# philbull/FastBox

Hardware: AMD Instinct MI355X
Metric: 512^3 box realisations/sec (gen + log-normal + P(k)) (higher is better)
Workload: dtype f32; 1 GPU; 512^3 Gaussian box (device Philox4x32-10 noise, stand-in EH P(k), L=1000 Mpc) + log-normal transform + binned P(k), nbins=20; nsamp=512, parallelism=replicas x1, streams_per_gpu=2, warmup_steps_run=5, spin_up_steps=160, full=False

## Files before the change

fastbox_amd/_lib.py:

```python
import ctypes
import os
import subprocess

_HERE = os.path.dirname(os.path.abspath(__file__))
LIB_PATH = os.environ.get("FASTBOX_HIP_LIB") or os.path.join(_HERE, "lib", "libfastbox_hip.so")
CSRC = os.path.join(_HERE, "csrc")

c_void_p, c_int, c_double, c_size_t = ctypes.c_void_p, ctypes.c_int, ctypes.c_double, ctypes.c_size_t
c_u64, c_i64 = ctypes.c_uint64, ctypes.c_int64
P_double = ctypes.POINTER(ctypes.c_double)
P_i32 = ctypes.POINTER(ctypes.c_int32)

SIGNATURES = {
    "fb_version": (c_int, []),
    "fb_last_error": (ctypes.c_char_p, []),
    "fb_plan_create": (c_int, [ctypes.POINTER(c_void_p), c_int, c_double, c_double, c_double, c_int, c_int,
                               P_double, P_double, P_double, P_double]),
    "fb_plan_destroy": (c_int, [c_void_p]),
    "fb_half_pitch": (c_int, [c_void_p]),
    "fb_half_rows": (c_int, [c_void_p]),
    "fb_real_bytes": (c_i64, [c_void_p]),
    "fb_half_bytes": (c_i64, [c_void_p]),
    "fb_full_bytes": (c_i64, [c_void_p]),
    "fb_fft_c2c": (c_int, [c_void_p, c_void_p, c_int, c_double, c_void_p]),
# ... 157 lines not shown
    "fb_slab_z_pass": (c_int, [c_void_p, c_void_p, c_void_p, c_int, c_int, c_int, c_void_p, c_void_p]),
    "fb_slab_x_bin_chunk": (c_int, [c_void_p, c_void_p, c_int, c_int, c_int, c_int, c_int, c_int, c_void_p, c_void_p]),
    "fb_set_plane_batching": (c_int, [c_void_p, c_int, c_int]),
    "fb_set_pass_schedule": (c_int, [c_void_p, c_int, c_int, c_int]),
    "fb_set_tile_rows": (c_int, [c_void_p, c_int]),
    "fb_comm_unique_id": (c_int, [c_void_p]),
    "fb_comm_create": (c_int, [c_void_p, c_int, c_int, c_void_p]),
    "fb_comm_destroy": (c_int, [c_void_p]),
    "fb_comm_info": (c_int, [c_void_p, P_i32, P_i32, P_i32]),
    "fb_slab_exchange_begin": (c_int, [c_void_p, c_void_p, c_void_p, c_i64, c_void_p, P_i32]),
    "fb_slab_exchange_wait": (c_int, [c_void_p, c_int, c_void_p]),
    "fb_slab_exchange": (c_int, [c_void_p, c_void_p, c_void_p, c_i64, c_void_p]),
    "fb_allreduce_f64": (c_int, [c_void_p, c_void_p, c_int, c_int, c_void_p]),
    "fb_set_exp_shift": (c_int, [c_void_p, ctypes.c_double]),
    "fb_debug_pair_flush": (c_int, [c_i64]),
    "fb_debug_strided_pass": (c_int, [c_void_p, c_void_p, c_int, c_int, c_void_p]),
    "fb_debug_read_stamps": (c_int, [c_void_p, ctypes.POINTER(ctypes.c_longlong), c_i64]),
    "fb_profile_select": (c_int, [c_void_p, ctypes.c_uint]),
    "fb_profile_sample": (c_int, [c_void_p, c_int, ctypes.POINTER(c_i64)]),
    "fb_profile_start": (c_int, [c_void_p]),
    "fb_profile_stop": (c_int, [c_void_p, c_void_p, P_double, ctypes.POINTER(c_i64), c_int]),
    "fb_malloc": (c_int, [ctypes.POINTER(c_void_p), c_size_t]),
    "fb_free": (c_int, [c_void_p]),
    "fb_memcpy_h2d": (c_int, [c_void_p, c_void_p, c_size_t, c_void_p]),
    "fb_memcpy_d2h": (c_int, [c_void_p, c_void_p, c_size_t, c_void_p]),
    "fb_memcpy_d2d": (c_int, [c_void_p, c_void_p, c_size_t, c_void_p]),
    "fb_stream_create": (c_int, [ctypes.POINTER(c_void_p)]),
    "fb_stream_create_priority": (c_int, [ctypes.POINTER(c_void_p), c_int]),
    "fb_stream_destroy": (c_int, [c_void_p]),
    "fb_stream_sync": (c_int, [c_void_p]),
# ... 83 lines not shown
```

fastbox_amd/csrc/fb_api.hip:

```cpp
#include "../../include/fastbox_hip.h"
#include "fb_plan.h"
#include "fb_api_util.h"
#include "fb_kshell.h"
#include <dlfcn.h>
#include <rccl/rccl.h>
#include <algorithm>
#include <cmath>
#include <cstdio>
#include <cstdlib>
#include <cstring>
#include <vector>

static thread_local std::string g_last_error;

void fb_set_error(const std::string& msg) { g_last_error = msg; }

int fb_hip_check(hipError_t e, const char* what) {
    if (e == hipSuccess) return FB_OK;
    g_last_error = std::string(what) + ": " + hipGetErrorString(e);
    (void)hipGetLastError();
    return e == hipErrorOutOfMemory ? FB_ERR_NOMEM : FB_ERR_HIP;
}

namespace {
template <typename B, typename T> int upload(B& dst, const T* src, size_t n) {
    FB_TRY(dst.ensure(n * sizeof(T)));
    FB_HIP(hipMemcpy(dst, src, n * sizeof(T), hipMemcpyHostToDevice));
    return FB_OK;
}
template <typename T> int make_twiddles(FbBuf<>& out, int N) {
    std::vector<T> h((size_t)2 * N);
    for (int j = 0; j < N; ++j) {
        const long double a = -2.0L * 3.14159265358979323846264338327950288L * (long double)j / (long double)N;
        h[2 * (size_t)j] = (T)cosl(a);
        h[2 * (size_t)j + 1] = (T)sinl(a);
    }
    return upload(out, h.data(), h.size());
}
}

extern "C" {

int fb_version(void) { return 102; }
const char* fb_last_error(void) { return g_last_error.c_str(); }

int fb_device_count(int* count) {
    FB_REQUIRE(count, "null pointer");
    FB_HIP(hipGetDeviceCount(count));
    return FB_OK;
}

int fb_device_get(int* device) {
    FB_REQUIRE(device, "null pointer");
// ... 110 lines not shown
    FB_QUIESCE();
    p->amp_dense = nullptr;
    return FB_DISPATCH(p, fbi_set_amp_shells_f32(p, amp, nshell), fbi_set_amp_shells_f64(p, amp, nshell));
}
int fb_set_amplitude_sym(fb_plan* p, const double* amp, int64_t n) {
    FB_REQUIRE(p && amp, "null pointer");
    FB_USE_DEVICE(p);
    FB_QUIESCE();
    return FB_DISPATCH(p, fbi_set_amp_sym_f32(p, amp, n), fbi_set_amp_sym_f64(p, amp, n));
}
int fb_set_amplitude_dense(fb_plan* p, const void* amp_dev) {
    FB_REQUIRE(p && amp_dev, "null pointer");
    FB_USE_DEVICE(p);
    FB_QUIESCE();
    p->amp_dense = amp_dev;
    return FB_OK;
}
int fb_colour_noise(fb_plan* p, const void* re, const void* im, void* out, void* stream) {
    FB_REQUIRE(p && re && im && out, "null pointer");
    FB_USE_DEVICE(p);
    hipStream_t s = (hipStream_t)stream;
    return FB_DISPATCH(p, fbi_colour_noise_f32(p, re, im, out, s), fbi_colour_noise_f64(p, re, im, out, s));
}
int fb_colour_device(fb_plan* p, uint64_t seed, uint64_t realisation, void* out, void* stream) {
    FB_REQUIRE(p && out, "null pointer");
    FB_USE_DEVICE(p);
    hipStream_t s = (hipStream_t)stream;
    return FB_DISPATCH(p, fbi_colour_device_f32(p, seed, realisation, out, s),
                       fbi_colour_device_f64(p, seed, realisation, out, s));
}
// ... 577 lines not shown

int64_t fb_slab_half_bytes(const fb_plan* p, int nparts) {
    return (p && nparts > 0) ? (int64_t)(p->N / nparts) * p->NR * p->NZP * 2 * p->prec : 0;
}
int64_t fb_slab_kspace_bytes(const fb_plan* p, int nparts) {
    return (p && nparts > 0) ? (int64_t)p->N * (p->N / nparts) * p->NZP * 2 * p->prec : 0;
}

int fb_debug_strided_pass(fb_plan* p, void* half, int axis, int mode, void* stream) {
    FB_REQUIRE(p && half, "null pointer");
    FB_USE_DEVICE(p);
    hipStream_t s = (hipStream_t)stream;
    return FB_DISPATCH(p, fbi_debug_pass_f32(p, half, axis, mode, s), fbi_debug_pass_f64(p, half, axis, mode, s));
}

int fb_set_pass_schedule(fb_plan* p, int plain, int generator, int binning) {
    FB_REQUIRE(p, "null pointer");
    FB_REQUIRE(plain >= -1 && plain <= 1 && generator >= -1 && generator <= 1 && binning >= -1 && binning <= 1,
               "schedule: 0 (one workgroup per tile), 1 (resident workgroups) or -1 (by grid size)");
    p->pass_schedule[0] = plain; p->pass_schedule[1] = generator; p->pass_schedule[2] = binning;
    return FB_OK;
}
int fb_set_tile_rows(fb_plan* p, int bytes) {
    FB_REQUIRE(p, "null pointer");
    FB_REQUIRE(bytes == 0 || bytes == 64 || bytes == 128, "row segment of the strided passes' tiles: 0 (default), 64 or 128 bytes");
    p->wide_rows = bytes == 0 ? -1 : (bytes == 64 ? 0 : 7);
    return FB_OK;
}
int fb_set_exp_shift(fb_plan* p, double shift) {
    FB_REQUIRE(p, "null pointer");
// ... 120 lines not shown
```

fastbox_amd/csrc/fb_fft_kernels.h:

```cpp
#pragma once
#include <type_traits>
#include "fb_fft.h"
#include "fb_field_kernels.h"

namespace fb {

#ifndef FB_E16_FROM
#define FB_E16_FROM 2048
#endif
constexpr int strided_elems(int n) { return n >= FB_E16_FROM ? 16 : fb_min(8, n); }

#ifndef FB_TILE_LINE
#define FB_TILE_LINE 128
#endif
template <typename T> constexpr int tile_cols(int n) {
    return fb_max(fb_max(2, fb_min(FB_TILE_LINE / (2 * (int)sizeof(T)),
                                   (n >= FB_E16_FROM ? (sizeof(T) == 8 ? 65536 : 131072) : 65536) / (n * 2 * (int)sizeof(T)))),
                  64 / (n / strided_elems(n)));
}

template <typename T> constexpr int strided_wg_per_cu(int n) {
    const int tile = n * tile_cols<T>(n) * 2 * (int)sizeof(T), nt = tile_cols<T>(n) * (n / strided_elems(n));
    return fb_max(1, fb_min(2048 / nt, tile > 81920 ? 1 : tile > 36864 ? 2 : 4));
}
// ... 57 lines not shown
    long long stride;
    long long outer_stride;
    int ncols;
    T scale;
    int ntx;
    int ntiles;
    int drop_io;
    int wide;
    int ntx_shift;
    long long out_outer_stride;
    long long blk_stride;
    int blk_in, blk_out, blk_shift;
    int packed;
    int tile0;
    long long out_stride;
};

template <typename T> struct StridedOp {
    KGeom g;
    AmpSrc<T> amp;
    RngKey key;
    const int* thr;
    const double* bins;
    double* partial;
    long long partial_stride;
    cx<T>* plane_out;
    int nbins, namb, store;
    int outer0;
    int vel_on, vel_comp;
    double vel_fac;
// ... 102 lines not shown
#pragma unroll
        for (int r = 0; r < 4; ++r)
            if (r * 64 < op.nbins) {
                int th;
                if constexpr (PERSIST) th = lthr[r * 64 + (tid & 63)];
                else th = thrv[r];
                b += __builtin_popcountll(__ballot(th <= n2));
            }
        return b;
    };
    [[maybe_unused]] const int rot_rows = (int)gridDim.x >= a.ntx ? (int)gridDim.x / a.ntx : 1;
    auto place = [&](int id, int& bx, int& by) {
        const bool p2 = a.ntx_shift >= 0;
        bx = p2 ? (id & (a.ntx - 1)) : id % a.ntx;
        by = p2 ? (id >> a.ntx_shift) : id / a.ntx;
#ifndef FB_NO_TILE_ROTATE
        int rot = bx + by;
        if constexpr (PERSIST) rot += by / rot_rows;
        bx = p2 ? (rot & (a.ntx - 1)) : rot % a.ntx;
#endif
#ifndef FB_NO_XCD_PAIR
        if constexpr (TZ * sizeof(cx<T>) < 128) {
            constexpr int LPT = 128 / (TZ * (int)sizeof(cx<T>)), G = 8 * LPT;
            const int lg = bx % G;
            if (bx - lg + G <= a.ntx) bx = (bx - lg) + LPT * (lg % 8) + lg / 8;
        }
#endif
        bx += a.tile0;
    };
    int tile_id = blockIdx.x;
#ifndef FB_GEN_PARK
#define FB_GEN_PARK 16
#endif
// ... 66 lines not shown
                if (has_plane) {
                    asm volatile("");
                    plane = (kz == 0) || (kz == H);
                    flip = plane && ky > H;
                    kyd = flip ? N - ky : ky;
                }
                cx<T> wl[ACC ? NJ : 1], wh[ACC ? NJ : 1];
                auto lo = [&](int j) -> cx<T>& { if constexpr (ACC) return wl[j - J0]; else return v[j]; };
                auto hi = [&](int j) -> cx<T>& { if constexpr (ACC) return wh[j - J0]; else return v[j + E2]; };
                T A0[NJ], A1[NJ];
                auto A0v = [&](int j) -> T { return A0[j - J0]; };
                auto A1v = [&](int j) -> T { return A1[j - J0]; };
                {
                    const T pf = (T)0.70710678118654752440;
                    if (op.amp.sym) {
                        const long long sym_step = (long long)TPL * (H + 1) * op.g.NZP;
                        const T* sym0 = op.amp.sym + ((long long)t * (H + 1) + amy) * op.g.NZP + kz;
                        const T* sym1 = op.amp.sym + ((long long)(H - t) * (H + 1) + amy) * op.g.NZP + kz;
#pragma unroll
                        for (int j = J0; j < J0 + NJ; ++j) {
#ifdef FB_EXPERIMENT_NOAMP
                            A0[j - J0] = pf; A1[j - J0] = pf;
#else
                            A0[j - J0] = sym0[j * sym_step] * pf;
                            A1[j - J0] = sym1[-j * sym_step] * pf;
#endif
                        }
                    } else if (op.amp.shell) {
                        const int c2 = my * my + kz * kz;
#pragma unroll
                        for (int j = J0; j < J0 + NJ; ++j) {
                            const int kx = t + j * TPL, mh = kx - H;
                            A0[j - J0] = op.amp.shell[kx * kx + c2] * pf;
// ... 780 lines not shown
```

fastbox_amd/csrc/fb_fft_launch.inc:

```
#include <cstdlib>
#include <cstring>
#include "fb_plan.h"
#include "fb_fft_kernels.h"
#include "fb_fft_generic.h"

namespace {

using namespace fb;
typedef FB_REAL real_t;
typedef cx<real_t> cplx_t;

template <typename K> int set_lds(K kernel, size_t bytes) {
    if (bytes > 65536)
        FB_HIP(hipFuncSetAttribute(reinterpret_cast<const void*>(kernel),
                                   hipFuncAttributeMaxDynamicSharedMemorySize, (int)bytes));
    return FB_OK;
}

KGeom fft_geom(const fb_plan* p) { return KGeom{p->axis2, p->ksc, p->kpar, p->N, p->NZV, p->NZP, p->NR}; }
int gen_amplitude(const fb_plan* p, StridedOp<real_t>& op) {
    op.amp.shell = (p->amp_dense || p->amp_sym_only) ? nullptr : p->amp_shell.as<const real_t>();
    op.amp.dense = p->amp_sym_only ? nullptr : reinterpret_cast<const real_t*>(p->amp_dense);
    op.amp.sym = (op.amp.shell || p->amp_sym_only) ? p->amp_sym.as<const real_t>() : nullptr;
    if (!op.amp.shell && !op.amp.dense && !op.amp.sym) { fb_set_error("amplitude table not set (fb_set_amplitude_*)"); return FB_ERR_STATE; }
    return FB_OK;
}

template <int N, int MODE, int PERSIST, bool BLK>
int launch_strided_npb(fb_plan* p, const StridedArgs<real_t>& a, int nouter, int sign, StridedOp<real_t>& op,
                       hipStream_t s) {
    constexpr bool SPLIT = strided_split<real_t>(N, MODE, BLK);
    constexpr int E = strided_elems_of<real_t>(N, MODE, BLK), TPL = N / E, TZ = tile_cols_of<real_t>(N, MODE, BLK);
    constexpr int NW = (TZ * TPL + 63) / 64;
    size_t lds = (size_t)N * TZ * (SPLIT ? sizeof(real_t) : sizeof(cplx_t)) + (size_t)N * sizeof(cplx_t);
    if (smode_bins(MODE)) lds += (size_t)NW * 2 * op.nbins * sizeof(double) + (size_t)((op.nbins + 63) & ~63) * sizeof(int);
    StridedArgs<real_t> b = a;
    b.ntx = a.ntx ? a.ntx : (a.ncols + TZ - 1) / TZ;
    b.ntiles = b.ntx * nouter;
    b.ntx_shift = -1;
    for (int q = 0; q < 30; ++q) if ((1 << q) == b.ntx) b.ntx_shift = q;
    b.wide = ((long long)(E - 1) * TPL * a.stride * (long long)sizeof(cplx_t) >= 0xE0000000LL) ? 1 : 0;
    b.drop_io = p->debug_no_mem;
    auto pick = [&]() {
#ifndef FB_CSIGN_FROM
#define FB_CSIGN_FROM (1 << 30)
#endif
        if constexpr (MODE == SMODE_PLAIN && (strided_row128<real_t>(N, MODE, BLK) || N >= (FB_CSIGN_FROM)))
            return sign < 0 ? k_fft_strided<real_t, N, MODE, PERSIST, BLK, -1> : k_fft_strided<real_t, N, MODE, PERSIST, BLK, +1>;
        else return k_fft_strided<real_t, N, MODE, PERSIST, BLK>;
    };
    auto kernel = pick();
    int r = set_lds(kernel, lds);
    if (r) return r;
    int nblk = b.ntiles;
    if (PERSIST) {
        static thread_local int per_cu = 0;
        static thread_local size_t per_cu_lds = 0;
// ... 630 lines not shown
}

int FB_CAT(fbi_debug_pass_, FB_SUFFIX)(fb_plan* p, void* half, int axis, int mode, hipStream_t s) {
    const int N = p->N;
    cplx_t* h = reinterpret_cast<cplx_t*>(half);
    const bool packed = use_packed(p) && mode % 10 != 2;
    StridedArgs<real_t> a = axis == 0 ? half_x(p, h, packed) : half_y(p, h, packed);
    StridedOp<real_t> op = {};
    op.g = fft_geom(p);
    p->debug_no_mem = (mode >= 10);
    mode %= 10;
    struct Reset { fb_plan* q; ~Reset() { q->debug_no_mem = 0; } } reset{p};
    if (mode == 1) {
        op.amp.shell = p->amp_shell.as<const real_t>();
        op.amp.dense = nullptr;
        op.amp.sym = p->amp_sym.as<const real_t>();
        if (!op.amp.shell) { fb_set_error("amplitude shells not set"); return FB_ERR_STATE; }
#ifdef FB_STAMPS
        {
            int r = p->bin_partials.ensure(((size_t)N * 64 * 32 + 4096) * sizeof(double));
            if (r) return r;
            op.bins = p->bin_partials;
        }
#endif
        return launch_strided<SMODE_GEN>(p, N, a, N, +1, op, s);
    }
    if (mode == 2) {
        if (!p->nbins || !p->use_thr) { fb_set_error("bins not set"); return FB_ERR_STATE; }
        op.thr = p->thr; op.bins = p->bins; op.nbins = p->nbins; op.namb = p->namb; op.store = 0;
        for (int q = 0; q < 8; ++q) op.amb[q] = p->amb[q];
        return launch_strided<SMODE_BIN>(p, N, a, N, -1, op, s);
// ... 121 lines not shown
    r = slab_blocking(ao, p, nxl, nparts, true);
    if (r) return r;
    return launch_plain(p, N, ao, nxl, -1, s);
}

int FB_CAT(fbi_slab_x_pass_, FB_SUFFIX)(fb_plan* p, void* kslab, int nyl, int sign, hipStream_t s) {
    return launch_plain(p, p->N, slab_x(p, reinterpret_cast<cplx_t*>(kslab), nyl), nyl, sign, s);
}

int FB_CAT(fbi_slab_x_generate_, FB_SUFFIX)(fb_plan* p, void* kslab, int nyl, int ky0, uint64_t seed, uint64_t real,
                                            hipStream_t s) {
    StridedOp<real_t> op = {};
    op.g = fft_geom(p);
    op.amp.shell = p->amp_shell.as<const real_t>();
    if (!op.amp.shell || p->amp_dense) { fb_set_error("slab generation needs shell amplitudes (cubic box)"); return FB_ERR_STATE; }
    op.amp.sym = p->amp_sym.as<const real_t>();
    op.key.k[0] = (uint32_t)seed; op.key.k[1] = (uint32_t)(seed >> 32);
    op.key.k[2] = (uint32_t)real; op.key.k[3] = (uint32_t)(real >> 32);
    op.outer0 = ky0;
    return launch_strided<SMODE_GEN>(p, p->N, slab_x(p, reinterpret_cast<cplx_t*>(kslab), nyl), nyl, +1, op, s);
}

int FB_CAT(fbi_slab_x_bin_, FB_SUFFIX)(fb_plan* p, void* kslab, int nyl, int ky0, double* results, hipStream_t s) {
    if (!p->nbins || !p->use_thr) { fb_set_error("fused P(k) needs shell thresholds (fb_set_bins with thr)"); return FB_ERR_STATE; }
    const int nb = p->nbins;
    StridedOp<real_t> op = {};
    op.g = fft_geom(p);
    op.thr = p->thr; op.bins = p->bins; op.nbins = nb; op.namb = p->namb; op.store = 0; op.outer0 = ky0;
    for (int q = 0; q < 8; ++q) op.amb[q] = p->amb[q];
    int r = launch_strided<SMODE_BIN>(p, p->N, slab_x(p, reinterpret_cast<cplx_t*>(kslab), nyl), nyl, -1, op, s);
    if (r) return r;
// ... 15 lines not shown
int slab_blocking_chunk(StridedArgs<real_t>& a, const fb_plan* p, int nxl, int nparts, long long W, bool out_side) {
    const int N = p->N, E = strided_elems(N);
    int m = E / nparts, shift = 0;
    if (nparts < 1 || m * nparts != E) { fb_set_error("fused slab exchange needs the rank count to divide the points per thread"); return FB_ERR_UNSUPPORTED; }
    while ((1 << shift) < m) ++shift;
    const long long nyl = N / nparts;
    a.blk_shift = shift;
    a.blk_stride = (long long)nxl * nyl * W;
    if (out_side) { a.blk_out = 1; a.out_stride = W; a.out_outer_stride = nyl * W; }
    else { a.blk_in = 1; a.out_stride = p->NZP; a.out_outer_stride = (long long)p->NR * p->NZP; a.stride = W; a.outer_stride = nyl * W; }
    return FB_OK;
}
}

int FB_CAT(fbi_slab_tile_cols_, FB_SUFFIX)(const fb_plan* p) { return slab_tz(p->N); }

int FB_CAT(fbi_slab_x_generate_chunk_, FB_SUFFIX)(fb_plan* p, void* kchunk, int nyl, int ky0, uint64_t seed, uint64_t real,
                                                  int tile0, int ntile, hipStream_t s) {
    const int TZ = slab_tz(p->N);
    const long long W = (long long)ntile * TZ;
    StridedOp<real_t> op = {};
    op.g = fft_geom(p);
    op.amp.shell = p->amp_shell.as<const real_t>();
    if (!op.amp.shell || p->amp_dense) { fb_set_error("slab generation needs shell amplitudes (cubic box)"); return FB_ERR_STATE; }
    op.amp.sym = p->amp_sym.as<const real_t>();
    op.key.k[0] = (uint32_t)seed; op.key.k[1] = (uint32_t)(seed >> 32);
    op.key.k[2] = (uint32_t)real; op.key.k[3] = (uint32_t)(real >> 32);
    op.outer0 = ky0;
    cplx_t* k = reinterpret_cast<cplx_t*>(kchunk) - (long long)tile0 * TZ;
    StridedArgs<real_t> a{k, k, p->tw.as<const cplx_t>(), (long long)nyl * W, W, p->NZV, (real_t)1};
    a.ntx = ntile; a.tile0 = tile0;
    return launch_strided<SMODE_GEN>(p, p->N, a, nyl, +1, op, s);
}

int FB_CAT(fbi_slab_y_inverse_chunk_, FB_SUFFIX)(fb_plan* p, const void* recv_chunk, void* half_local, int nxl, int nparts,
                                                 int tile0, int ntile, hipStream_t s) {
    const int TZ = slab_tz(p->N);
    const long long W = (long long)ntile * TZ;
    cplx_t* h = reinterpret_cast<cplx_t*>(half_local);
    StridedArgs<real_t> a = slab_y(p, h);
// ... 92 lines not shown
```

fastbox_amd/csrc/fb_field_kernels.h:

```cpp
#pragma once
#include "fb_dev.h"
#include "fb_fft.h"
#include "fb_kshell.h"
#include "fb_rng.h"

namespace fb {

__device__ __forceinline__ int mirror_of(int i, int N) { return i == 0 ? 0 : N - i; }

struct KGeom {
    const double* axis2;
    const double* ksc;
    const double* kpar;
    int N, NZV, NZP;
    int NR;
};

__device__ __forceinline__ void fb_sincospi(float x, float* s, float* c) { sincospif(x, s, c); }
__device__ __forceinline__ void fb_sincospi(double x, double* s, double* c) { sincospi(x, s, c); }
__device__ __forceinline__ void fb_sincos(float x, float* s, float* c) { sincosf(x, s, c); }
__device__ __forceinline__ void fb_sincos(double x, double* s, double* c) { sincos(x, s, c); }

__device__ __forceinline__ double kmag_exact(const KGeom& g, int i, int j, int l) {
#pragma clang fp contract(off)
// ... 11 lines not shown
}

template <typename T> __device__ __forceinline__ T nan_to_num(T v) {
    if (v != v) return (T)0;
    if (sizeof(T) == 4) { if (v > (T)3.4028234663852886e38) return (T)3.4028234663852886e38;
                          if (v < (T)-3.4028234663852886e38) return (T)-3.4028234663852886e38; }
    else { if (v > (T)1.7976931348623157e308) return (T)1.7976931348623157e308;
           if (v < (T)-1.7976931348623157e308) return (T)-1.7976931348623157e308; }
    return v;
}

template <typename T> struct AmpSrc {
    const T* shell;
    const T* dense;
    const T* sym;
};
template <typename T>
__global__ void k_build_amp_sym(const T* __restrict__ shell, T* __restrict__ sym, int N, int NZP) {
    const int M = (N >> 1) + 1;
    const int c = blockIdx.x * blockDim.x + threadIdx.x;
    const int b = blockIdx.y, a = blockIdx.z;
    if (c >= NZP) return;
    sym[((long long)a * M + b) * NZP + c] = c < M ? shell[a * a + b * b + c * c] : (T)0;
}
template <typename T>
__device__ __forceinline__ T amp_at(const AmpSrc<T>& a, const KGeom& g, int i, int j, int l) {
    if (a.shell) return a.shell[shell_of(i, j, l, g.N)];
    if (a.sym) {
        const int mi = mode_of(i, g.N), mj = mode_of(j, g.N), ml = mode_of(l, g.N);
        const int M = (g.N >> 1) + 1;
        return a.sym[((long long)(mi < 0 ? -mi : mi) * M + (mj < 0 ? -mj : mj)) * g.NZP + (ml < 0 ? -ml : ml)];
    }
    return a.dense[((long long)i * g.NR + j) * g.NZP + l];
}

template <typename T>
__global__ void k_colour_noise(const T* __restrict__ re, const T* __restrict__ im, cx<T>* __restrict__ out,
                               AmpSrc<T> amp, KGeom g) {
    const int N = g.N;
    const int l = blockIdx.x * blockDim.x + threadIdx.x;
    const int j = blockIdx.y, i = blockIdx.z;
    if (l >= g.NZV) return;
    const long long a = ((long long)i * N + j) * N + l;
    const long long b = ((long long)mirror_of(i, N) * N + mirror_of(j, N)) * N + mirror_of(l, N);
    const T A = (T)0.5 * amp_at(amp, g, i, j, l);
    out[((long long)i * g.NR + j) * g.NZP + l] = cx<T>{A * (re[a] + re[b]), A * (im[a] - im[b])};
// ... 1322 lines not shown
```

fastbox_amd/csrc/fb_field_launch.inc:

```
#include <algorithm>
#include <cmath>
#include <cstdlib>
#include "fb_plan.h"
#include "fb_api_util.h"
#include "fb_field_kernels.h"
#include <vector>

namespace {
using namespace fb;
typedef FB_REAL real_t;
typedef cx<real_t> cplx_t;

KGeom geom(const fb_plan* p) { return KGeom{p->axis2, p->ksc, p->kpar, p->N, p->NZV, p->NZP, p->NR}; }
BinGeom bin_geom(const fb_plan* p) {
    BinGeom b;
    b.bins = p->bins; b.thr = p->use_thr ? p->thr : nullptr; b.nbins = p->nbins; b.namb = p->namb;
    for (int q = 0; q < 8; ++q) b.amb[q] = p->amb[q];
    return b;
}
dim3 mode_grid(const fb_plan* p, int nz, int bs) { return dim3((nz + bs - 1) / bs, p->N, p->N); }
RngKey rng_key(uint64_t seed, uint64_t real) {
    RngKey k;
    k.k[0] = (uint32_t)seed; k.k[1] = (uint32_t)(seed >> 32); k.k[2] = (uint32_t)real; k.k[3] = (uint32_t)(real >> 32);
    return k;
}
dim3 row_grid(const fb_plan* p) {
    return dim3((unsigned)(((long long)p->N * p->N + FB_ROW_GROUPS - 1) / FB_ROW_GROUPS));
}
int mode_block(int nz) {
    int best = 64;
    for (int bs = 128; bs <= 256; bs <<= 1)
        if ((nz + bs - 1) / bs * bs <= (nz + best - 1) / best * best) best = bs;
    return best;
}

int amp_src(const fb_plan* p, AmpSrc<real_t>& a) {
    a.shell = p->amp_shell.as<const real_t>();
    a.dense = reinterpret_cast<const real_t*>(p->amp_dense);
    a.sym = p->amp_sym.as<const real_t>();
    if (a.dense) a.shell = nullptr;
    if (p->amp_sym_only) { a.shell = nullptr; a.dense = nullptr; }
    if (!a.shell && !a.dense && !a.sym) { fb_set_error("amplitude table not set (fb_set_amplitude_*)"); return FB_ERR_STATE; }
    return FB_OK;
}
}

#define FB_CAT2(a, b) a##b
#define FB_CAT(a, b) FB_CAT2(a, b)
#define FBI(name) FB_CAT(FB_CAT(fbi_, name), FB_CAT(_, FB_SUFFIX))

int FBI(set_amp_shells)(fb_plan* p, const double* amp, int64_t n) {
    std::vector<real_t> tmp((size_t)n);
    for (int64_t q = 0; q < n; ++q) tmp[(size_t)q] = (real_t)amp[q];
    FB_TRY(p->amp_shell.reset());
    FB_TRY(p->amp_shell.ensure((size_t)n * sizeof(real_t)));
    FB_HIP(hipMemcpy(p->amp_shell, tmp.data(), (size_t)n * sizeof(real_t), hipMemcpyHostToDevice));
    p->nshell = n;
    p->amp_sym_only = 0;
    const int N = p->N, M = N / 2 + 1;
    if (const char* e = getenv("FB_NO_AMP_SYM")) if (e[0] == '1') {
        return p->amp_sym.reset();
    }
    if (n < (int64_t)3 * (N / 2) * (N / 2) + 1) { fb_set_error("shell table shorter than 3 (N/2)^2 + 1"); return FB_ERR_INVALID; }
    FB_TRY(p->amp_sym.ensure((size_t)M * M * p->NZP * sizeof(real_t)));
    hipLaunchKernelGGL((k_build_amp_sym<real_t>), dim3((p->NZP + 63) / 64, M, M), dim3(64), 0, 0,
                       p->amp_shell.as<const real_t>(), p->amp_sym.as<real_t>(), N, p->NZP);
    FB_LAUNCH_CHECK("k_build_amp_sym");
    FB_HIP(hipDeviceSynchronize());
    return FB_OK;
}

int FBI(set_amp_sym)(fb_plan* p, const double* amp, int64_t n) {
    const int N = p->N, M = N / 2 + 1;
    if (n != (int64_t)M * M * M) { fb_set_error("expected (N/2+1)^3 amplitudes"); return FB_ERR_INVALID; }
    std::vector<real_t> tmp((size_t)M * M * p->NZP, (real_t)0);
    for (int a = 0; a < M; ++a)
        for (int b = 0; b < M; ++b)
            for (int c = 0; c < M; ++c)
                tmp[((size_t)a * M + b) * p->NZP + c] = (real_t)amp[((size_t)a * M + b) * M + c];
    FB_TRY(p->amp_sym.ensure(tmp.size() * sizeof(real_t)));
    FB_HIP(hipMemcpy(p->amp_sym, tmp.data(), tmp.size() * sizeof(real_t), hipMemcpyHostToDevice));
    p->amp_sym_only = 1;
    p->amp_dense = nullptr;
    return FB_OK;
}

int FBI(colour_noise)(fb_plan* p, const void* re, const void* im, void* out, hipStream_t s) {
    AmpSrc<real_t> a;
    int r = amp_src(p, a);
    if (r) return r;
    const int bs = mode_block(p->NZV);
    { FbProfScope _ps(p, FBK_COLOUR, s);
    hipLaunchKernelGGL((k_colour_noise<real_t>), mode_grid(p, p->NZV, bs), dim3(bs), 0, s,
                       (const real_t*)re, (const real_t*)im, (cplx_t*)out, a, geom(p)); }
    FB_LAUNCH_CHECK("k_colour_noise");
    return FB_OK;
// ... 434 lines not shown
```

fastbox_amd/csrc/fb_plan.h:

```cpp
#pragma once
#include <hip/hip_runtime.h>
#include <stdint.h>
#include "fb_keyed_cache.h"
#include <string>
#include <vector>

#define FB_OK 0
#define FB_ERR_INVALID -1
#define FB_ERR_HIP -2
#define FB_ERR_UNSUPPORTED -3
#define FB_ERR_NOMEM -4
#define FB_ERR_STATE -5
#define FB_ERR_RCCL -6

void fb_set_error(const std::string& msg);
int fb_hip_check(hipError_t e, const char* what);
#define FB_HIP(x) do { int _r = fb_hip_check((x), #x); if (_r) return _r; } while (0)
#define FB_TRY(x) do { const int _r = (x); if (_r) return _r; } while (0)
#define FB_LAUNCH_CHECK(name) do { int _r = fb_hip_check(hipGetLastError(), name); if (_r) return _r; } while (0)

template <typename T = void> struct FbBuf {
    T* ptr = nullptr;
    size_t cap = 0;
    FbBuf() = default;
// ... 6 lines not shown
    int ensure(size_t need) { return cap >= need ? FB_OK : grow(need); }
    int reset() {
        T* q = ptr;
        ptr = nullptr; cap = 0;
        if (q) FB_HIP(hipFree(q));
        return FB_OK;
    }
private:
    __attribute__((noinline)) int grow(size_t need) {
        FB_TRY(reset());
        FB_HIP(hipMalloc(reinterpret_cast<void**>(&ptr), need));
        cap = need;
        return FB_OK;
    }
};

struct fb_comm;

struct fb_cyl_rows {
    int nb = 0;
    FbBuf<int> rows_dev;
    std::vector<int> off;
    std::vector<double> sumk;
    bool has0 = false;
};

struct fb_plan {
    fb_comm* comm = nullptr;
    int N = 0;
    int generic = 0;
// ... 13 lines not shown
    int cubic = 0;

    FbBuf<> tw;
    FbBuf<double> axis2;
    FbBuf<double> kpar;
    FbBuf<double> ksc;
    FbBuf<double> zgrid;

    FbBuf<> amp_shell;
    int64_t nshell = 0;
    const void* amp_dense = nullptr;
    FbBuf<> work;
    FbBuf<double> eig_work;
    FbBuf<double> kperp_tab;
    int amp_sym_only = 0;
    FbBuf<> amp_sym;

    FbBuf<double> bins;
    int nbins = 0;
    FbBuf<int> thr;
    int use_thr = 0;
    int namb = 0;
    int amb[8] = {0, 0, 0, 0, 0, 0, 0, 0};
    FbBuf<unsigned long long> counts;
    double counts_host[256];
    FbBuf<double> partials;
    int prow = 0;
    FbBuf<double> scratch;
    FbBuf<double> bin_partials;
    long long bin_rows = 0;
    long long bin_rows_main = 0;
// ... 129 lines not shown
                                double scale, hipStream_t s); \
    int fbi_power_fused_##sfx(fb_plan* p, const void* real_in, void* work_half, int pre_exp, int store, \
                              double* results, hipStream_t s); \
    int fbi_debug_pass_##sfx(fb_plan* p, void* half, int axis, int mode, hipStream_t s); \
    int fbi_realise_begin_##sfx(fb_plan* p, uint64_t seed, uint64_t real, void* work_half, hipStream_t s); \
    int fbi_realise_finish_##sfx(fb_plan* p, void* work_half, void* real_out, double scale, hipStream_t s); \
    int fbi_power_from_pending_##sfx(fb_plan* p, void* work_half, void* real_out, double scale, int pre_exp, \
                                     double* results, hipStream_t s); \
    int fbi_slab_forward_local_##sfx(fb_plan* p, const void* real_local, void* half_local, int nxl, int pre_exp, \
                                     double* expsum, hipStream_t s); \
    int fbi_slab_inverse_local_##sfx(fb_plan* p, void* half_local, void* real_local, int nxl, double scale, hipStream_t s); \
    int fbi_slab_x_pass_##sfx(fb_plan* p, void* kslab, int nyl, int sign, hipStream_t s); \
    int fbi_slab_x_generate_##sfx(fb_plan* p, void* kslab, int nyl, int ky0, uint64_t seed, uint64_t real, hipStream_t s); \
    int fbi_slab_x_bin_##sfx(fb_plan* p, void* kslab, int nyl, int ky0, double* results, hipStream_t s); \
    int fbi_slab_tile_cols_##sfx(const fb_plan* p); \
    int fbi_slab_x_generate_chunk_##sfx(fb_plan* p, void* kchunk, int nyl, int ky0, uint64_t seed, uint64_t real, int tile0, \
                                        int ntile, hipStream_t s); \
    int fbi_slab_y_inverse_chunk_##sfx(fb_plan* p, const void* recv_chunk, void* half_local, int nxl, int nparts, int tile0, \
                                       int ntile, hipStream_t s); \
    int fbi_slab_y_forward_chunk_##sfx(fb_plan* p, const void* half_local, void* send_chunk, int nxl, int nparts, int tile0, \
                                       int ntile, hipStream_t s); \
    int fbi_slab_z_pass_##sfx(fb_plan* p, void* half_local, void* real_local, int nxl, int which, double scale, int pre_exp, \
                              double* expsum, hipStream_t s); \
    int fbi_slab_x_bin_chunk_##sfx(fb_plan* p, void* kchunk, int nyl, int ky0, int tile0, int ntile, int first, int last, \
                                   double* results, hipStream_t s);
FB_DECL(f32)
FB_DECL(f64)
int fbi_bin_count(fb_plan* p, hipStream_t s);
int fbi_slab_permute(fb_plan* p, const void* in, void* out, int nxl, int nparts, int pack, hipStream_t s);
```

include/fastbox_hip.h:

```cpp
#ifndef FASTBOX_HIP_H
#define FASTBOX_HIP_H

#include <stddef.h>
#include <stdint.h>

#ifdef __cplusplus
extern "C" {
#endif

#define FB_OK 0
#define FB_ERR_INVALID -1
#define FB_ERR_HIP -2
#define FB_ERR_UNSUPPORTED -3
#define FB_ERR_NOMEM -4
#define FB_ERR_STATE -5
#define FB_ERR_RCCL -6

typedef struct fb_plan fb_plan;

int fb_version(void);
const char* fb_last_error(void);

int fb_plan_create(fb_plan** plan, int N, double Lx, double Ly, double Lz, int precision, int device,
                   const double* axis2, const double* ksc, const double* kpar, const double* zgrid);
// ... 320 lines not shown
int fb_comm_unique_id(void* id128);
int fb_comm_create(fb_plan* plan, int world, int rank, const void* id128);
int fb_comm_destroy(fb_plan* plan);
int fb_comm_info(const fb_plan* plan, int* world, int* rank, int* rccl_version);
int fb_slab_exchange_begin(fb_plan* plan, const void* send, void* recv, int64_t bytes_per_peer, void* stream, int* ticket);
int fb_slab_exchange_wait(fb_plan* plan, int ticket, void* stream);
int fb_slab_exchange(fb_plan* plan, const void* send, void* recv, int64_t bytes_per_peer, void* stream);
int fb_allreduce_f64(fb_plan* plan, double* data_dev, int count, int op, void* stream);

int fb_set_plane_batching(fb_plan* plan, int planes, int streams);
int fb_set_pass_schedule(fb_plan* plan, int plain, int generator, int binning);
int fb_set_tile_rows(fb_plan* plan, int bytes);
int fb_set_exp_shift(fb_plan* plan, double shift);
int fb_debug_strided_pass(fb_plan* plan, void* half, int axis, int mode, void* stream);
int fb_debug_pair_flush(int64_t pairs);
int fb_debug_read_stamps(fb_plan* plan, long long* host, int64_t count);

int fb_malloc(void** dev_ptr, size_t bytes);
int fb_free(void* dev_ptr);
int fb_memcpy_h2d(void* dst_dev, const void* src_host, size_t bytes, void* stream);
int fb_memcpy_d2h(void* dst_host, const void* src_dev, size_t bytes, void* stream);
int fb_memcpy_d2d(void* dst_dev, const void* src_dev, size_t bytes, void* stream);
int fb_stream_create(void** stream);
int fb_stream_create_priority(void** stream, int priority);
int fb_stream_destroy(void* stream);
int fb_stream_sync(void* stream);
int fb_stream_wait_stream(void* waiter, void* signaller);
int fb_device_count(int* count);
int fb_device_get(int* device);
int fb_device_set(int device);
// ... 6 lines not shown
```

Before: 1051 boxes/s.

## Block amplitude symmetry table by tile columns, pair mirrored generator rows, share tables

Reorders the symmetric amplitude table into blocks of z-columns matched to the generator tile width, so that the mirrored t and H-t lookups hit contiguous short runs. The generator also schedules tile rows q and N-q in adjacent groups of eight tiles, so both mirror halves of a row reuse the same amplitude block in cache. A process-wide registry, keyed by hash, deduplicates identical amplitude tables across plans (for example across replicas), which saves device memory and L2 footprint. The cost is a more complex indexing scheme, a host-side hash of the shell table, and a new scheduling path that only runs when its divisibility conditions are met.

```diff
diff --git a/fastbox_amd/_lib.py b/fastbox_amd/_lib.py
--- a/fastbox_amd/_lib.py
+++ b/fastbox_amd/_lib.py
@@ -195,6 +195,7 @@
     "fb_allreduce_f64": (c_int, [c_void_p, c_void_p, c_int, c_int, c_void_p]),
     "fb_set_exp_shift": (c_int, [c_void_p, ctypes.c_double]),
     "fb_debug_pair_flush": (c_int, [c_i64]),
+    "fb_debug_amp_tables": (c_int, [ctypes.POINTER(c_i64)]),
     "fb_debug_strided_pass": (c_int, [c_void_p, c_void_p, c_int, c_int, c_void_p]),
     "fb_debug_read_stamps": (c_int, [c_void_p, ctypes.POINTER(ctypes.c_longlong), c_i64]),
     "fb_profile_select": (c_int, [c_void_p, ctypes.c_uint]),
diff --git a/fastbox_amd/csrc/fb_api.hip b/fastbox_amd/csrc/fb_api.hip
--- a/fastbox_amd/csrc/fb_api.hip
+++ b/fastbox_amd/csrc/fb_api.hip
@@ -37,6 +37,11 @@
     }
     return upload(out, h.data(), h.size());
 }
+}
+
+FbSharedRegistry<fb_amp_table>& fb_amp_registry() {
+    static FbSharedRegistry<fb_amp_table>* r = new FbSharedRegistry<fb_amp_table>();
+    return *r;
 }
 
 extern "C" {
@@ -177,6 +182,7 @@
     FB_USE_DEVICE(p);
     FB_QUIESCE();
     p->amp_dense = amp_dev;
+    if (!p->amp_sym_only) p->amp_sym.reset();
     return FB_OK;
 }
 int fb_colour_noise(fb_plan* p, const void* re, const void* im, void* out, void* stream) {
@@ -784,6 +790,12 @@
     return FB_DISPATCH(p, fbi_debug_pass_f32(p, half, axis, mode, s), fbi_debug_pass_f64(p, half, axis, mode, s));
 }
 
+int fb_debug_amp_tables(int64_t* tables) {
+    FB_REQUIRE(tables, "null pointer");
+    *tables = (int64_t)fb_amp_registry().live();
+    return FB_OK;
+}
+
 int fb_set_pass_schedule(fb_plan* p, int plain, int generator, int binning) {
     FB_REQUIRE(p, "null pointer");
     FB_REQUIRE(plain >= -1 && plain <= 1 && generator >= -1 && generator <= 1 && binning >= -1 && binning <= 1,
diff --git a/fastbox_amd/csrc/fb_fft_kernels.h b/fastbox_amd/csrc/fb_fft_kernels.h
--- a/fastbox_amd/csrc/fb_fft_kernels.h
+++ b/fastbox_amd/csrc/fb_fft_kernels.h
@@ -95,6 +95,7 @@
     int packed;
     int tile0;
     long long out_stride;
+    int pair_rows;
 };
 
 template <typename T> struct StridedOp {
@@ -227,9 +228,21 @@
         const bool p2 = a.ntx_shift >= 0;
         bx = p2 ? (id & (a.ntx - 1)) : id % a.ntx;
         by = p2 ? (id >> a.ntx_shift) : id / a.ntx;
+        [[maybe_unused]] int rk = by, rks = by;
+#ifndef FB_NO_GEN_MIRROR_PAIR
+        if constexpr (MODE == SMODE_GEN) {
+            if (a.pair_rows) {
+                const int u = ((id >> 4) << 3) | (id & 7), w = (id >> 3) & 1;
+                const int q = p2 ? (u >> a.ntx_shift) : u / a.ntx;
+                bx = p2 ? (u & (a.ntx - 1)) : u % a.ntx;
+                by = q ? (w ? N - q : q) : (w ? N / 2 : 0);
+                rk = q; rks = 2 * q;
+            }
+        }
+#endif
 #ifndef FB_NO_TILE_ROTATE
-        int rot = bx + by;
-        if constexpr (PERSIST) rot += by / rot_rows;
+        int rot = bx + rk;
+        if constexpr (PERSIST) rot += rks / rot_rows;
         bx = p2 ? (rot & (a.ntx - 1)) : rot % a.ntx;
 #endif
 #ifndef FB_NO_XCD_PAIR
@@ -326,9 +339,12 @@
                 {
                     const T pf = (T)0.70710678118654752440;
                     if (op.amp.sym) {
-                        const long long sym_step = (long long)TPL * (H + 1) * op.g.NZP;
-                        const T* sym0 = op.amp.sym + ((long long)t * (H + 1) + amy) * op.g.NZP + kz;
-                        const T* sym1 = op.amp.sym + ((long long)(H - t) * (H + 1) + amy) * op.g.NZP + kz;
+                        const int bs = op.amp.sym_bs;
+                        const long long sym_step = (long long)TPL << bs;
+                        const long long blk = ((long long)amy * (op.g.NZP >> bs) + (kz >> bs)) * (H + 1);
+                        const int kzl = kz & ((1 << bs) - 1);
+                        const T* sym0 = op.amp.sym + (((blk + t) << bs) + kzl);
+                        const T* sym1 = op.amp.sym + (((blk + (H - t)) << bs) + kzl);
 #pragma unroll
                         for (int j = J0; j < J0 + NJ; ++j) {
 #ifdef FB_EXPERIMENT_NOAMP
diff --git a/fastbox_amd/csrc/fb_fft_launch.inc b/fastbox_amd/csrc/fb_fft_launch.inc
--- a/fastbox_amd/csrc/fb_fft_launch.inc
+++ b/fastbox_amd/csrc/fb_fft_launch.inc
@@ -21,7 +21,8 @@
 int gen_amplitude(const fb_plan* p, StridedOp<real_t>& op) {
     op.amp.shell = (p->amp_dense || p->amp_sym_only) ? nullptr : p->amp_shell.as<const real_t>();
     op.amp.dense = p->amp_sym_only ? nullptr : reinterpret_cast<const real_t*>(p->amp_dense);
-    op.amp.sym = (op.amp.shell || p->amp_sym_only) ? p->amp_sym.as<const real_t>() : nullptr;
+    op.amp.sym = (op.amp.shell || p->amp_sym_only) ? p->sym<real_t>() : nullptr;
+    op.amp.sym_bs = p->sym_bs();
     if (!op.amp.shell && !op.amp.dense && !op.amp.sym) { fb_set_error("amplitude table not set (fb_set_amplitude_*)"); return FB_ERR_STATE; }
     return FB_OK;
 }
@@ -41,6 +42,7 @@
     for (int q = 0; q < 30; ++q) if ((1 << q) == b.ntx) b.ntx_shift = q;
     b.wide = ((long long)(E - 1) * TPL * a.stride * (long long)sizeof(cplx_t) >= 0xE0000000LL) ? 1 : 0;
     b.drop_io = p->debug_no_mem;
+    b.pair_rows = (MODE == SMODE_GEN && nouter == N && op.outer0 == 0 && b.ntiles % 16 == 0) ? 1 : 0;
     auto pick = [&]() {
 #ifndef FB_CSIGN_FROM
 #define FB_CSIGN_FROM (1 << 30)
@@ -701,7 +703,8 @@
     if (mode == 1) {
         op.amp.shell = p->amp_shell.as<const real_t>();
         op.amp.dense = nullptr;
-        op.amp.sym = p->amp_sym.as<const real_t>();
+        op.amp.sym = p->sym<real_t>();
+        op.amp.sym_bs = p->sym_bs();
         if (!op.amp.shell) { fb_set_error("amplitude shells not set"); return FB_ERR_STATE; }
 #ifdef FB_STAMPS
         {
@@ -853,7 +856,8 @@
     op.g = fft_geom(p);
     op.amp.shell = p->amp_shell.as<const real_t>();
     if (!op.amp.shell || p->amp_dense) { fb_set_error("slab generation needs shell amplitudes (cubic box)"); return FB_ERR_STATE; }
-    op.amp.sym = p->amp_sym.as<const real_t>();
+    op.amp.sym = p->sym<real_t>();
+    op.amp.sym_bs = p->sym_bs();
     op.key.k[0] = (uint32_t)seed; op.key.k[1] = (uint32_t)(seed >> 32);
     op.key.k[2] = (uint32_t)real; op.key.k[3] = (uint32_t)(real >> 32);
     op.outer0 = ky0;
@@ -899,6 +903,16 @@
 }
 
 int FB_CAT(fbi_slab_tile_cols_, FB_SUFFIX)(const fb_plan* p) { return slab_tz(p->N); }
+int FB_CAT(fbi_gen_tile_cols_, FB_SUFFIX)(const fb_plan* p) {
+    if (p->generic) return 0;
+    switch (p->N) {
+#define FB_GEN_TZ_CASE(N_) case N_: return tile_cols_of<real_t>(N_, SMODE_GEN, false);
+        FB_GEN_TZ_CASE(16) FB_GEN_TZ_CASE(32) FB_GEN_TZ_CASE(64) FB_GEN_TZ_CASE(128) FB_GEN_TZ_CASE(256) FB_GEN_TZ_CASE(512)
+        FB_GEN_TZ_CASE(1024) FB_GEN_TZ_CASE(2048)
+#undef FB_GEN_TZ_CASE
+    }
+    return 0;
+}
 
 int FB_CAT(fbi_slab_x_generate_chunk_, FB_SUFFIX)(fb_plan* p, void* kchunk, int nyl, int ky0, uint64_t seed, uint64_t real,
                                                   int tile0, int ntile, hipStream_t s) {
@@ -908,7 +922,8 @@
     op.g = fft_geom(p);
     op.amp.shell = p->amp_shell.as<const real_t>();
     if (!op.amp.shell || p->amp_dense) { fb_set_error("slab generation needs shell amplitudes (cubic box)"); return FB_ERR_STATE; }
-    op.amp.sym = p->amp_sym.as<const real_t>();
+    op.amp.sym = p->sym<real_t>();
+    op.amp.sym_bs = p->sym_bs();
     op.key.k[0] = (uint32_t)seed; op.key.k[1] = (uint32_t)(seed >> 32);
     op.key.k[2] = (uint32_t)real; op.key.k[3] = (uint32_t)(real >> 32);
     op.outer0 = ky0;
diff --git a/fastbox_amd/csrc/fb_field_kernels.h b/fastbox_amd/csrc/fb_field_kernels.h
--- a/fastbox_amd/csrc/fb_field_kernels.h
+++ b/fastbox_amd/csrc/fb_field_kernels.h
@@ -49,22 +49,25 @@
     const T* shell;
     const T* dense;
     const T* sym;
+    int sym_bs;
 };
-template <typename T>
-__global__ void k_build_amp_sym(const T* __restrict__ shell, T* __restrict__ sym, int N, int NZP) {
+__device__ __forceinline__ long long amp_sym_index(int a, int b, int c, int M, int NZP, int bs) {
+    return ((((long long)b * (NZP >> bs) + (c >> bs)) * M + a) << bs) + (c & ((1 << bs) - 1));
+}
+template <typename T>
+__global__ void k_build_amp_sym(const T* __restrict__ shell, T* __restrict__ sym, int N, int NZP, int bs) {
     const int M = (N >> 1) + 1;
     const int c = blockIdx.x * blockDim.x + threadIdx.x;
     const int b = blockIdx.y, a = blockIdx.z;
     if (c >= NZP) return;
-    sym[((long long)a * M + b) * NZP + c] = c < M ? shell[a * a + b * b + c * c] : (T)0;
+    sym[amp_sym_index(a, b, c, M, NZP, bs)] = c < M ? shell[a * a + b * b + c * c] : (T)0;
 }
 template <typename T>
 __device__ __forceinline__ T amp_at(const AmpSrc<T>& a, const KGeom& g, int i, int j, int l) {
     if (a.shell) return a.shell[shell_of(i, j, l, g.N)];
     if (a.sym) {
         const int mi = mode_of(i, g.N), mj = mode_of(j, g.N), ml = mode_of(l, g.N);
-        const int M = (g.N >> 1) + 1;
-        return a.sym[((long long)(mi < 0 ? -mi : mi) * M + (mj < 0 ? -mj : mj)) * g.NZP + (ml < 0 ? -ml : ml)];
+        return a.sym[amp_sym_index(mi < 0 ? -mi : mi, mj < 0 ? -mj : mj, ml < 0 ? -ml : ml, (g.N >> 1) + 1, g.NZP, a.sym_bs)];
     }
     return a.dense[((long long)i * g.NR + j) * g.NZP + l];
 }
diff --git a/fastbox_amd/csrc/fb_field_launch.inc b/fastbox_amd/csrc/fb_field_launch.inc
--- a/fastbox_amd/csrc/fb_field_launch.inc
+++ b/fastbox_amd/csrc/fb_field_launch.inc
@@ -1,6 +1,7 @@
 #include <algorithm>
 #include <cmath>
 #include <cstdlib>
+#include <cstring>
 #include "fb_plan.h"
 #include "fb_api_util.h"
 #include "fb_field_kernels.h"
@@ -37,7 +38,8 @@
 int amp_src(const fb_plan* p, AmpSrc<real_t>& a) {
     a.shell = p->amp_shell.as<const real_t>();
     a.dense = reinterpret_cast<const real_t*>(p->amp_dense);
-    a.sym = p->amp_sym.as<const real_t>();
+    a.sym = p->sym<real_t>();
+    a.sym_bs = p->sym_bs();
     if (a.dense) a.shell = nullptr;
     if (p->amp_sym_only) { a.shell = nullptr; a.dense = nullptr; }
     if (!a.shell && !a.dense && !a.sym) { fb_set_error("amplitude table not set (fb_set_amplitude_*)"); return FB_ERR_STATE; }
@@ -48,6 +50,20 @@
 #define FB_CAT2(a, b) a##b
 #define FB_CAT(a, b) FB_CAT2(a, b)
 #define FBI(name) FB_CAT(FB_CAT(fbi_, name), FB_CAT(_, FB_SUFFIX))
+
+namespace {
+int amp_block_shift(const fb_plan* p) {
+    int tz = FBI(gen_tile_cols)(p), bs = 0;
+    if (tz < 1 || tz > 16) tz = 16;
+    while ((2 << bs) <= tz) ++bs;
+    return bs;
+}
+std::shared_ptr<fb_amp_table> new_amp_table(const fb_plan* p, int bs) {
+    std::shared_ptr<fb_amp_table> e = std::make_shared<fb_amp_table>();
+    e->device = p->device; e->N = p->N; e->NZP = p->NZP; e->prec = p->prec; e->bs = bs;
+    return e;
+}
+}
 
 int FBI(set_amp_shells)(fb_plan* p, const double* amp, int64_t n) {
     std::vector<real_t> tmp((size_t)n);
@@ -59,27 +75,53 @@
     p->amp_sym_only = 0;
     const int N = p->N, M = N / 2 + 1;
     if (const char* e = getenv("FB_NO_AMP_SYM")) if (e[0] == '1') {
-        return p->amp_sym.reset();
+        p->amp_sym.reset();
+        return FB_OK;
     }
     if (n < (int64_t)3 * (N / 2) * (N / 2) + 1) { fb_set_error("shell table shorter than 3 (N/2)^2 + 1"); return FB_ERR_INVALID; }
-    FB_TRY(p->amp_sym.ensure((size_t)M * M * p->NZP * sizeof(real_t)));
-    hipLaunchKernelGGL((k_build_amp_sym<real_t>), dim3((p->NZP + 63) / 64, M, M), dim3(64), 0, 0,
-                       p->amp_shell.as<const real_t>(), p->amp_sym.as<real_t>(), N, p->NZP);
-    FB_LAUNCH_CHECK("k_build_amp_sym");
-    FB_HIP(hipDeviceSynchronize());
+    const int bs = amp_block_shift(p);
+    const size_t bytes = (size_t)n * sizeof(real_t);
+    const uint64_t hash = fb_hash_bytes(tmp.data(), bytes);
+    int r = FB_OK;
+    std::shared_ptr<fb_amp_table> t = fb_amp_registry().acquire(
+        [&](const fb_amp_table& e) {
+            return e.device == p->device && e.N == N && e.NZP == p->NZP && e.prec == p->prec && e.bs == bs && e.hash == hash &&
+                   e.shell.size() == bytes && memcmp(e.shell.data(), tmp.data(), bytes) == 0;
+        },
+        [&]() -> std::shared_ptr<fb_amp_table> {
+            std::shared_ptr<fb_amp_table> e = new_amp_table(p, bs);
+            r = [&]() -> int {
+                FB_TRY(e->sym.ensure(fb_amp_table::elems(N, p->NZP) * sizeof(real_t)));
+                FB_HIP(hipMemsetAsync(e->sym.as<real_t>() + (size_t)M * M * p->NZP, 0, (size_t)64 * M * sizeof(real_t), 0));
+                hipLaunchKernelGGL((k_build_amp_sym<real_t>), dim3((p->NZP + 63) / 64, M, M), dim3(64), 0, 0,
+                                   p->amp_shell.as<const real_t>(), e->sym.as<real_t>(), N, p->NZP, bs);
+                FB_LAUNCH_CHECK("k_build_amp_sym");
+                FB_HIP(hipDeviceSynchronize());
+                return FB_OK;
+            }();
+            if (r) return nullptr;
+            e->hash = hash;
+            e->shell.assign(reinterpret_cast<const unsigned char*>(tmp.data()), reinterpret_cast<const unsigned char*>(tmp.data()) + bytes);
+            return e;
+        });
+    if (!t) return r ? r : FB_ERR_NOMEM;
+    p->amp_sym = std::move(t);
     return FB_OK;
 }
 
 int FBI(set_amp_sym)(fb_plan* p, const double* amp, int64_t n) {
     const int N = p->N, M = N / 2 + 1;
     if (n != (int64_t)M * M * M) { fb_set_error("expected (N/2+1)^3 amplitudes"); return FB_ERR_INVALID; }
-    std::vector<real_t> tmp((size_t)M * M * p->NZP, (real_t)0);
+    const int bs = amp_block_shift(p);
+    std::vector<real_t> tmp(fb_amp_table::elems(N, p->NZP), (real_t)0);
     for (int a = 0; a < M; ++a)
         for (int b = 0; b < M; ++b)
             for (int c = 0; c < M; ++c)
-                tmp[((size_t)a * M + b) * p->NZP + c] = (real_t)amp[((size_t)a * M + b) * M + c];
-    FB_TRY(p->amp_sym.ensure(tmp.size() * sizeof(real_t)));
-    FB_HIP(hipMemcpy(p->amp_sym, tmp.data(), tmp.size() * sizeof(real_t), hipMemcpyHostToDevice));
+                tmp[fb_amp_table::index(N, p->NZP, bs, a, b, c)] = (real_t)amp[((size_t)a * M + b) * M + c];
+    std::shared_ptr<fb_amp_table> e = new_amp_table(p, bs);
+    FB_TRY(e->sym.ensure(tmp.size() * sizeof(real_t)));
+    FB_HIP(hipMemcpy(e->sym, tmp.data(), tmp.size() * sizeof(real_t), hipMemcpyHostToDevice));
+    p->amp_sym = std::move(e);
     p->amp_sym_only = 1;
     p->amp_dense = nullptr;
     return FB_OK;
diff --git a/fastbox_amd/csrc/fb_plan.h b/fastbox_amd/csrc/fb_plan.h
--- a/fastbox_amd/csrc/fb_plan.h
+++ b/fastbox_amd/csrc/fb_plan.h
@@ -2,6 +2,8 @@
 #include <hip/hip_runtime.h>
 #include <stdint.h>
 #include "fb_keyed_cache.h"
+#include "fb_shared_registry.h"
+#include <memory>
 #include <string>
 #include <vector>
 
@@ -44,6 +46,19 @@
         return FB_OK;
     }
 };
+
+struct fb_amp_table {
+    int device = 0, N = 0, NZP = 0, prec = 0, bs = 0;
+    uint64_t hash = 0;
+    std::vector<unsigned char> shell;
+    FbBuf<> sym;
+    static size_t elems(int N, int NZP) { return ((size_t)(N / 2 + 1) * NZP + 64) * (size_t)(N / 2 + 1); }
+    static size_t index(int N, int NZP, int bs, int a, int b, int c) {
+        return ((((size_t)b * (size_t)(NZP >> bs) + (size_t)(c >> bs)) * (size_t)(N / 2 + 1) + (size_t)a) << bs) + (size_t)(c & ((1 << bs) - 1));
+    }
+};
+
+FbSharedRegistry<fb_amp_table>& fb_amp_registry();
 
 struct fb_comm;
 
@@ -87,7 +102,9 @@
     FbBuf<double> eig_work;
     FbBuf<double> kperp_tab;
     int amp_sym_only = 0;
-    FbBuf<> amp_sym;
+    std::shared_ptr<fb_amp_table> amp_sym;
+    template <typename U> const U* sym() const { return amp_sym ? amp_sym->sym.as<const U>() : nullptr; }
+    int sym_bs() const { return amp_sym ? amp_sym->bs : 0; }
 
     FbBuf<double> bins;
     int nbins = 0;
@@ -247,6 +264,7 @@
     int fbi_slab_x_generate_##sfx(fb_plan* p, void* kslab, int nyl, int ky0, uint64_t seed, uint64_t real, hipStream_t s); \
     int fbi_slab_x_bin_##sfx(fb_plan* p, void* kslab, int nyl, int ky0, double* results, hipStream_t s); \
     int fbi_slab_tile_cols_##sfx(const fb_plan* p); \
+    int fbi_gen_tile_cols_##sfx(const fb_plan* p); \
     int fbi_slab_x_generate_chunk_##sfx(fb_plan* p, void* kchunk, int nyl, int ky0, uint64_t seed, uint64_t real, int tile0, \
                                         int ntile, hipStream_t s); \
     int fbi_slab_y_inverse_chunk_##sfx(fb_plan* p, const void* recv_chunk, void* half_local, int nxl, int nparts, int tile0, \
diff --git a/fastbox_amd/csrc/fb_shared_registry.h b/fastbox_amd/csrc/fb_shared_registry.h
--- /dev/null
+++ b/fastbox_amd/csrc/fb_shared_registry.h
@@ -0,0 +1,42 @@
+#pragma once
+#include <cstddef>
+#include <cstdint>
+#include <memory>
+#include <mutex>
+#include <vector>
+
+template <typename V> class FbSharedRegistry {
+    std::mutex m_;
+    std::vector<std::weak_ptr<V>> e_;
+public:
+    template <typename Match, typename Make> std::shared_ptr<V> acquire(Match&& match, Make&& make) {
+        std::lock_guard<std::mutex> lock(m_);
+        size_t keep = 0;
+        std::shared_ptr<V> hit;
+        for (size_t q = 0; q < e_.size(); ++q) {
+            std::shared_ptr<V> s = e_[q].lock();
+            if (!s) continue;
+            if (!hit && match(static_cast<const V&>(*s))) hit = s;
+            if (keep != q) e_[keep] = std::move(e_[q]);
+            ++keep;
+        }
+        e_.resize(keep);
+        if (hit) return hit;
+        std::shared_ptr<V> made = make();
+        if (made) e_.push_back(made);
+        return made;
+    }
+    size_t live() {
+        std::lock_guard<std::mutex> lock(m_);
+        size_t n = 0;
+        for (const auto& w : e_) n += w.expired() ? 0 : 1;
+        return n;
+    }
+};
+
+inline uint64_t fb_hash_bytes(const void* data, size_t n) {
+    const unsigned char* b = static_cast<const unsigned char*>(data);
+    uint64_t h = 1469598103934665603ull;
+    for (size_t q = 0; q < n; ++q) { h ^= b[q]; h *= 1099511628211ull; }
+    return h;
+}
diff --git a/include/fastbox_hip.h b/include/fastbox_hip.h
--- a/include/fastbox_hip.h
+++ b/include/fastbox_hip.h
@@ -358,6 +358,7 @@
 int fb_set_exp_shift(fb_plan* plan, double shift);
 int fb_debug_strided_pass(fb_plan* plan, void* half, int axis, int mode, void* stream);
 int fb_debug_pair_flush(int64_t pairs);
+int fb_debug_amp_tables(int64_t* tables);
 int fb_debug_read_stamps(fb_plan* plan, long long* host, int64_t count);
 
 int fb_malloc(void** dev_ptr, size_t bytes);
```

Measured after the change: 1051 boxes/s, median of 2. About the same (+0.0%).
